# google-research/seed_rl

Hardware: NVIDIA H100
Metric: env-frames/sec (learner, device-timed) on synthetic 84x84x4 T=20 unrolls @1/2/4/8 H100 (higher is better)
Workload: dtype bf16x3 (fp32-faithful tensor-core contraction; activations stored as bf16 hi+lo pairs), f32 elsewhere

## Files before the change

include/seedrl_b200.h:

```cpp
#ifndef SEEDRL_B200_H_
#define SEEDRL_B200_H_

#include <stddef.h>
#include <stdint.h>

#ifdef __cplusplus
extern "C" {
#endif

#define SEEDRL_OK 0
#define SEEDRL_ERR_INVALID_ARGUMENT 3
#define SEEDRL_ERR_OUT_OF_RANGE 11
#define SEEDRL_ERR_INTERNAL 13
#define SEEDRL_ERR_CANCELLED 1
#define SEEDRL_ERR_UNAVAILABLE 14

typedef void* seedrl_stream_t;

const char* seedrl_last_error(void);
int seedrl_abi_version(void);
uint64_t seedrl_kernel_launch_count(void);

int seedrl_vtrace_from_importance_weights(
    int T, int B,
// ... 248 lines not shown
                       const float* B, int ldb, float* C, int ldc, const float* bias,
                       const float* mask, int ldm, int relu, int accumulate, int a_relu,
                       seedrl_stream_t stream);
int seedrl_debug_strided_conv(int op, int mode, int gather, int in_u8, int N, int H, int W, int C, int K,
                              int S, int cout, const void* x, const float* w, const float* bias,
                              const float* dy, const float* mask, float* out, int ldo, float* dbias,
                              float* col, size_t col_bytes, float* ws, size_t ws_bytes, int* error_flag,
                              int* gathered, seedrl_stream_t stream);
size_t seedrl_debug_lstm_workspace_bytes(int mode, int H, int T1, int B);
int seedrl_debug_lstm_forward(int mode, int gemm_mode, int H, int T1, int B, const float* U, const uint8_t* done,
                              float* z, const float* h0, const float* c0, float* hs, float* cs, float* hp,
                              void* ws, size_t ws_bytes, int* error_flag, seedrl_stream_t stream);
int seedrl_debug_lstm_backward(int mode, int gemm_mode, int H, int T1, int B, const float* U, const uint8_t* done,
                               const float* gates, const float* cs, const float* c0, const float* dhs, float* dz,
                               void* ws, size_t ws_bytes, int* error_flag, seedrl_stream_t stream);
int seedrl_debug_r2d2_net_views(const seedrl_r2d2_net* net, int T, int B, int index, size_t* offset, size_t* bytes);
int seedrl_debug_net_views(const seedrl_net* net, int T1, int B, int index, size_t* offset, size_t* bytes,
                           int* format);

size_t seedrl_debug_planes_bytes(int N, int H, int W, int C);
int seedrl_debug_to_planes(int N, int H, int W, int C, int relu, const float* x, void* out,
                           seedrl_stream_t stream);
int seedrl_debug_from_planes(int N, int H, int W, int C, const void* in, float* y,
                             seedrl_stream_t stream);
int seedrl_debug_convp(int cin, int cout, int N, int H, int W, const void* in, const float* w,
                       const float* bias, const void* mask, const void* res, int flip,
                       void* out_raw, void* out_relu, float* out_nhwc, void* wq_scratch,
                       int* error_flag, seedrl_stream_t stream);
int seedrl_debug_wgradp(int cin, int cout, int N, int H, int W, const void* x, const void* dy,
                        float* dw, float* db, float* partial, size_t partial_bytes,
                        int* error_flag, seedrl_stream_t stream);
int seedrl_debug_poolp(int backward, int N, int H, int W, int C, const void* in, void* out_raw,
                       void* out_relu, float* out_nhwc, uint8_t* idx, seedrl_stream_t stream);

#ifdef __cplusplus
}
#endif
#endif
```

seed_rl_b200/_lib.py:

```python
import ctypes
import os

_HERE = os.path.dirname(os.path.abspath(__file__))
LIB_PATH = os.path.join(_HERE, 'libseedrl_b200.so')

c_void_p, c_int, c_float, c_size_t = ctypes.c_void_p, ctypes.c_int, ctypes.c_float, ctypes.c_size_t
c_i64, c_u64 = ctypes.c_int64, ctypes.c_uint64
P = c_void_p


class SeedrlError(RuntimeError):

  def __init__(self, code, msg):
    super().__init__('libseedrl_b200 error %d: %s' % (code, msg))
    self.code = code


class LossConfig(ctypes.Structure):
  _fields_ = [('discounting', c_float), ('lambda_', c_float), ('baseline_cost', c_float),
              ('kl_cost', c_float), ('max_abs_reward', c_float),
              ('clip_rho_threshold', c_float), ('clip_pg_rho_threshold', c_float),
              ('target_entropy', c_float), ('has_target_entropy', ctypes.c_int32),
              ('entropy_cost_adjustment_speed', c_float)]

# ... 95 lines not shown
    'seedrl_r2d2_net_num_params': (c_size_t, [P]),
    'seedrl_r2d2_net_arena_floats': (c_size_t, [P]),
    'seedrl_r2d2_net_set_mode': (c_int, [P, c_int]),
    'seedrl_r2d2_net_set_lstm_mode': (c_int, [P, c_int]),
    'seedrl_r2d2_net_param_info':
        (c_int, [P, c_int, ctypes.c_char_p, c_size_t, ctypes.POINTER(c_i64), ctypes.POINTER(c_int),
                 ctypes.POINTER(c_size_t)]),
    'seedrl_r2d2_net_workspace_bytes': (c_size_t, [P, c_int, c_int]),
    'seedrl_r2d2_net_forward':
        (c_int, [P, P, c_int, c_int, P, P, P, P, P, P, P, P, P, P, P, c_size_t, P]),
    'seedrl_r2d2_net_backward': (c_int, [P, P, c_int, c_int, P, P, P, P, P, c_size_t, P]),
    'seedrl_r2d2_net_check_error': (c_int, [P, c_int, c_int, P, c_size_t, P]),
    'seedrl_r2d2_stack_frames': (c_int, [c_int, c_int, c_int, c_int, P, P, P, P, P, P]),
    'seedrl_r2d2_loss_scratch_bytes': (c_size_t, [c_int, c_int, c_int]),
    'seedrl_r2d2_loss_fwd_bwd': (c_int, [c_int, c_int, c_int, P, P, P, P, P, P, c_float, c_int, c_float, c_float,
                                         P, P, P, P, P]),
    'seedrl_r2d2_retrace_loss_scratch_bytes': (c_size_t, [c_int, c_int]),
    'seedrl_r2d2_retrace_loss_fwd_bwd': (c_int, [c_int, c_int, c_int, P, P, P, P, P, P, c_float, c_float, c_float,
                                                 c_float, P, P, P, P, P]),
    'seedrl_r2d2_epsilon_greedy': (c_int, [c_int, c_int, P, P, c_u64, P, P, P]),
    'seedrl_replay_sample': (c_int, [c_int, P, c_float, c_float, c_int, P, P, P, P, P]),
    'seedrl_clip_scratch_bytes': (c_size_t, []),
    'seedrl_clip_by_global_norm': (c_int, [c_size_t, P, c_float, P, P, P]),
    'seedrl_profile_num_categories': (c_int, []),
    'seedrl_profile_category_name': (ctypes.c_char_p, [c_int]),
    'seedrl_profile_begin': (c_int, [P]),
    'seedrl_profile_end': (c_int, [ctypes.POINTER(ctypes.c_double), ctypes.POINTER(c_u64)]),
    'seedrl_debug_planes_bytes': (c_size_t, [c_int, c_int, c_int, c_int]),
    'seedrl_debug_to_planes': (c_int, [c_int, c_int, c_int, c_int, c_int, P, P, P]),
    'seedrl_debug_from_planes': (c_int, [c_int, c_int, c_int, c_int, P, P, P]),
    'seedrl_debug_convp': (c_int, [c_int, c_int, c_int, c_int, c_int, P, P, P, P, P, c_int, P, P, P, P, P, P]),
    'seedrl_debug_wgradp': (c_int, [c_int, c_int, c_int, c_int, c_int, P, P, P, P, P, c_size_t, P, P]),
    'seedrl_debug_poolp': (c_int, [c_int, c_int, c_int, c_int, c_int, P, P, P, P, P, P]),
    'seedrl_debug_conv3x3': (c_int, [c_int, c_int, c_int, c_int, c_int, c_int, P, P, P, P, P, P, P]),
    'seedrl_debug_conv3x3_flip': (c_int, [c_int, c_int, P, P, P]),
    'seedrl_debug_conv3x3_tc':
        (c_int, [c_int, c_int, c_int, c_int, c_int, c_int, c_int, P, P, P, P, P, P, c_int, c_int, P, P, P]),
    'seedrl_debug_wgrad_partial_bytes': (c_size_t, []),
    'seedrl_debug_conv_pixels': (c_int, [c_int, c_int, c_int, c_int, c_int, c_int, P]),
    'seedrl_debug_set_loss_stream': (c_int, [c_int]),
    'seedrl_debug_set_wgrad_chunk': (c_int, [c_int]),
    'seedrl_debug_set_conv_tile': (c_int, [c_int]),
    'seedrl_debug_set_gemm_bk': (c_int, [c_int]),
    'seedrl_debug_set_first_layer_dense': (c_int, [c_int]),
    'seedrl_debug_conv0pool': (c_int, [c_int, c_int, c_int, P, P, P, P, P, P, P, P]),
    'seedrl_debug_conv0pool_c': (c_int, [c_int, c_int, c_int, c_int, P, P, P, P, P, P, P, P]),
    'seedrl_debug_first_wgrad_pooled_c': (c_int, [c_int, c_int, c_int, c_int, P, P, P, P, P, P, c_size_t, P]),
    'seedrl_debug_conv3x3_wgrad_tc':
        (c_int, [c_int, c_int, c_int, c_int, c_int, c_int, c_int, P, P, P, P, P, c_size_t, P, P]),
    'seedrl_debug_conv3x3_wgrad':
        (c_int, [c_int, c_int, c_int, c_int, c_int, c_int, P, P, P, P, P, c_size_t, P]),
    'seedrl_debug_maxpool': (c_int, [c_int, c_int, c_int, c_int, c_int, P, P, P, P]),
    'seedrl_debug_gemm_tc':
        (c_int, [c_int, c_int, c_int, c_int, c_int, c_int, P, c_int, P, c_int, P, c_int, P, P, c_int, c_int, c_int,
                 c_int, P, c_size_t, P, P]),
    'seedrl_debug_set_gemm_gather': (c_int, [c_int]),
    'seedrl_debug_colsum': (c_int, [c_int, c_int, P, c_int, P, P, c_size_t, P]),
    'seedrl_debug_sgemm':
        (c_int, [c_int, c_int, c_int, c_int, c_int, P, c_int, P, c_int, P, c_int, P, P, c_int,
                 c_int, c_int, c_int, P]),
    'seedrl_debug_strided_conv':
        (c_int, [c_int, c_int, c_int, c_int, c_int, c_int, c_int, c_int, c_int, c_int, c_int, P, P, P, P, P, P,
                 c_int, P, P, c_size_t, P, c_size_t, P, ctypes.POINTER(c_int), P]),
    'seedrl_debug_lstm_workspace_bytes': (c_size_t, [c_int, c_int, c_int, c_int]),
    'seedrl_debug_lstm_forward':
        (c_int, [c_int, c_int, c_int, c_int, c_int, P, P, P, P, P, P, P, P, P, c_size_t, P, P]),
# ... 60 lines not shown
```

seed_rl_b200/csrc/conv_planes.cu:

```cuda
#include <cuda.h>
#include <cuda_bf16.h>

#include <cstdio>
#include <cstdlib>

#include "kernels.h"
#include "tc_common.cuh"

namespace seedrl {

long long planes_positions(int N, int H, int W) {
  const long long Q = (long long)N * (H + 1) * (W + 2);
  return ((Q + 2 * (W + 2) + 2 + 256 + 127) / 128) * 128;
}
size_t planes_bytes(int N, int H, int W, int C) {
  return (size_t)planes_positions(N, H, W) * 16 * 2 * (C / 8);
}

typedef CUresult (*EncodeTiledFn)(CUtensorMap*, CUtensorMapDataType, cuuint32_t, void*, const cuuint64_t*,
                                  const cuuint64_t*, const cuuint32_t*, const cuuint32_t*,
                                  CUtensorMapInterleave, CUtensorMapSwizzle, CUtensorMapL2promotion,
                                  CUtensorMapFloatOOBfill);
static EncodeTiledFn encode_tiled_fn() {
  static EncodeTiledFn fn = nullptr;
// ... 64 lines not shown
  int nch;
  int chunk;
  int ntiles;
  int nb;
  const uint4* wq;
  const float* bias;
  const uint4* mask;
  const uint4* res;
  uint4* out_raw;
  uint4* out_relu;
  float* out_nhwc;
  int* err;
};

constexpr int kCpWarpgroups = 4;
constexpr int kCpThreads = 128 * kCpWarpgroups + 32;
constexpr int kCpM = 128;
constexpr int kCpMaxStages = 4;

__device__ __forceinline__ void quad_transpose(float2 (&t)[4], int q) {
#pragma unroll
  for (int b = 1; b <= 2; b <<= 1) {
    const bool up = (q & b) != 0;
#pragma unroll
    for (int u = 0; u < 4; ++u) {
      if (u & b) continue;
      const float2 send = up ? t[u] : t[u | b];
      const float2 r = make_float2(__shfl_xor_sync(0xffffffffu, send.x, b), __shfl_xor_sync(0xffffffffu, send.y, b));
      if (up) t[u] = r; else t[u | b] = r;
    }
  }
}

template <int CIN, int COUT, int NSUB>
__global__ void __launch_bounds__(kCpThreads, 1)
convp_kernel(const __grid_constant__ CUtensorMap tm_in, const ConvpArgs a) {
  constexpr int G = CIN / 8, GO = COUT / 8, NS = CIN / 16;
  constexpr int MT = NSUB * kCpM;
  constexpr int NBLK = 2 * NSUB;
  extern __shared__ __align__(128) uint8_t smem_raw[];
  const int PW = a.g.PW, nb = a.nb;
  const uint32_t P = (uint32_t)(a.nch * a.chunk) * 16u;
  const uint32_t stage_bytes = 2u * G * P;
  uint8_t* s_stage = smem_raw;
  uint4* s_b = reinterpret_cast<uint4*>(smem_raw + (size_t)nb * stage_bytes);
  float* s_bias = reinterpret_cast<float*>(s_b + 2 * 9 * CIN * COUT / 8);
  uint64_t* s_full = reinterpret_cast<uint64_t*>(s_bias + COUT);
  uint64_t* s_empty = s_full + kCpMaxStages;
  const int tid = threadIdx.x, warp = tid >> 5, lane = tid & 31;

  for (int i = tid; i < 2 * 9 * CIN * COUT / 8; i += kCpThreads) s_b[i] = __ldg(a.wq + i);
  if (tid < COUT) s_bias[tid] = a.bias ? __ldg(a.bias + tid) : 0.f;
  if (tid == 0) {
    for (int i = 0; i < nb; ++i) {
      mbar_init(s_full + i, 1);
      mbar_init(s_empty + i, 4 * kCpWarpgroups);
    }
    asm volatile("fence.mbarrier_init.release.cluster;" ::: "memory");
    asm volatile("prefetch.tensormap [%0];" ::"l"(reinterpret_cast<uint64_t>(&tm_in)) : "memory");
  }
  asm volatile("fence.proxy.async.shared::cta;" ::: "memory");
  __syncthreads();

  const int my_tiles = ((int)blockIdx.x < a.ntiles) ? (a.ntiles - 1 - (int)blockIdx.x) / (int)gridDim.x + 1 : 0;
  bool timed_out = false;

  if (warp == 4 * kCpWarpgroups) {
    if (elect_one()) {
      for (int it = 0; it < my_tiles; ++it) {
        const int s = it % nb;
// ... 1 lines not shown
        const int tile = (int)blockIdx.x + it * (int)gridDim.x;
        mbar_expect_tx(s_full + s, stage_bytes);
        tma_load_3d(s_stage + (size_t)s * stage_bytes, &tm_in, 0, tile * MT / a.chunk, 0, s_full + s);
      }
    }
    __syncwarp();
  } else {
    const int cw = warp >> 2;
    const size_t plane_u = (size_t)a.Lp;
    if (blockIdx.x == 0) {
      const uint4 z = make_uint4(0u, 0u, 0u, 0u);
      for (int i = tid; i < (PW + 1) * 2 * GO; i += 128 * kCpWarpgroups) {
        const int pl = i / (PW + 1), s = i - pl * (PW + 1);
        if (a.out_raw) a.out_raw[(size_t)pl * plane_u + s] = z;
        if (a.out_relu) a.out_relu[(size_t)pl * plane_u + s] = z;
      }
    }
    const int q = lane & 3;
    const int row = 16 * (warp & 3) + (lane >> 2) + 8 * (q & 1);
    const uint32_t b_base = smem_u32(s_b);
    const uint64_t db0 = gmma_desc(b_base, (uint32_t)(2 * GO) * 128u, 128u);
    for (int it = 0; it < my_tiles; ++it) {
      const int s = it % nb;
      const int tile = (int)blockIdx.x + it * (int)gridDim.x;
      if (!mbar_wait_bounded(s_full + s, (uint32_t)((it / nb) & 1))) { timed_out = true; break; }
      const int m0 = (cw - it * NBLK) & (kCpWarpgroups - 1);
      if (m0 >= NBLK && lane == 0) mbar_arrive(s_empty + s);
      const uint32_t a_base = smem_u32(s_stage + (size_t)s * stage_bytes);
      const uint64_t da0 = gmma_desc(a_base, P, 128u);
      const uint64_t lo_off = (uint64_t)((G * P) >> 4), slab_off = (uint64_t)((2 * P) >> 4);
#pragma unroll 1
      for (int m = m0; m < NBLK; m += kCpWarpgroups) {
        float acc[COUT];
#pragma unroll
        for (int i = 0; i < COUT; ++i) acc[i] = 0.f;
        wgmma_fence_acc<COUT>(acc);
        wgmma_fence();
#pragma unroll
        for (int tap = 0; tap < 9; ++tap) {
          const uint64_t off = (uint64_t)(m * 64 + (tap / 3) * PW + (tap % 3));
#pragma unroll
          for (int sl = 0; sl < NS; ++sl) {
            const uint64_t da = da0 + off + (uint64_t)sl * slab_off;
            const uint64_t db = db0 + (uint64_t)((tap * NS + sl) * (COUT * 64 / 16));
            Wgmma<2 * COUT>::template mma<0, 0>(acc, da, db, 1u);
            Wgmma<COUT>::template mma<0, 0>(acc, da + lo_off, db, 1u);
          }
        }
        wgmma_commit();
        const int p = tile * MT + m * 64 + row;
        const int sp = p + PW + 1;
        const int pix = out_pixel(a.g, p);
        uint4 mk[GO / 2], rh[GO / 2], rl[GO / 2];
        if (pix >= 0) {
#pragma unroll
          for (int k = 0; k < GO / 2; ++k) {
            const int go = (q >> 1) + 2 * k;
            if (a.mask) mk[k] = __ldg(a.mask + (size_t)go * plane_u + sp);
            if (a.res) {
              rh[k] = __ldg(a.res + (size_t)go * plane_u + sp);
              rl[k] = __ldg(a.res + (size_t)(GO + go) * plane_u + sp);
            }
          }
        }
        wgmma_wait<0>();
        wgmma_fence_acc<COUT>(acc);
        if (m + kCpWarpgroups >= NBLK && lane == 0) mbar_arrive(s_empty + s);
        const bool in_store = sp < a.Lp;
#pragma unroll
        for (int k = 0; k < GO / 2; ++k) {
          const int go = (q >> 1) + 2 * k;
          float2 t[4];
#pragma unroll
          for (int u = 0; u < 4; ++u) {
            const int j = 2 * k + (u >> 1), h = u & 1;
            t[u] = make_float2(acc[4 * j + 2 * h] + acc[4 * (j + GO) + 2 * h],
                               acc[4 * j + 2 * h + 1] + acc[4 * (j + GO) + 2 * h + 1]);
          }
          quad_transpose(t, q);
          float x[8];
#pragma unroll
          for (int e = 0; e < 4; ++e) {
// ... 320 lines not shown
  if (i >= (long long)Lp * G) return;
  const int s = (int)(i / G), go = (int)(i - (long long)s * G);
  const int pix = in_pixel(g, s);
  if (pix < 0) return;
  const uint4 h = __ldg(in + (size_t)go * Lp + s), l = __ldg(in + (size_t)(G + go) * Lp + s);
  float4* dst = reinterpret_cast<float4*>(y + (size_t)pix * (G * 8) + go * 8);
  dst[0] = make_float4(bf16lo(h.x) + bf16lo(l.x), bf16hi(h.x) + bf16hi(l.x), bf16lo(h.y) + bf16lo(l.y),
                       bf16hi(h.y) + bf16hi(l.y));
  dst[1] = make_float4(bf16lo(h.z) + bf16lo(l.z), bf16hi(h.z) + bf16hi(l.z), bf16lo(h.w) + bf16lo(l.w),
                       bf16hi(h.w) + bf16hi(l.w));
}

int to_planes(int N, int H, int W, int C, int relu, const float* x, void* out, cudaStream_t st) {
  const ConvGeom g = make_geom(N, H, W);
  const long long Lp = planes_positions(N, H, W);
  const long long n = Lp * (C / 8);
  to_planes_kernel<<<(unsigned)((n + 255) / 256), 256, 0, st>>>(g, (int)Lp, C / 8, relu, x,
                                                                reinterpret_cast<uint4*>(out));
  count_launch(PC_MISC, st);
  SEEDRL_CHECK_LAUNCH();
  return SEEDRL_OK;
}
int from_planes(int N, int H, int W, int C, const void* in, float* y, cudaStream_t st) {
  const ConvGeom g = make_geom(N, H, W);
  const long long Lp = planes_positions(N, H, W);
  const long long n = Lp * (C / 8);
  from_planes_kernel<<<(unsigned)((n + 255) / 256), 256, 0, st>>>(g, (int)Lp, C / 8,
                                                                  reinterpret_cast<const uint4*>(in), y);
  count_launch(PC_MISC, st);
  SEEDRL_CHECK_LAUNCH();
  return SEEDRL_OK;
}

__global__ void poolp_fwd_kernel(ConvGeom go_, int Lp, int G, int H, int W, int pt, int pl,
                                 const float* __restrict__ x, uint4* __restrict__ out_raw,
                                 uint4* __restrict__ out_relu, uint8_t* __restrict__ idx) {
  const long long i = (long long)blockIdx.x * blockDim.x + threadIdx.x;
  if (i >= (long long)Lp * G) return;
  const int s = (int)(i / G), gq = (int)(i - (long long)s * G);
  const int pix = in_pixel(go_, s);
  float best[8];
  unsigned char arg[8];
#pragma unroll
  for (int e = 0; e < 8; ++e) { best[e] = 0.f; arg[e] = 0; }
  if (pix >= 0) {
    const int Wo = go_.W, Ho = go_.H, C = G * 8;
    const int n = pix / (Ho * Wo), r = pix - n * (Ho * Wo), ho = r / Wo, wo = r - ho * Wo;
#pragma unroll
    for (int e = 0; e < 8; ++e) best[e] = -INFINITY;
#pragma unroll
    for (int kh = 0; kh < 3; ++kh) {
      const int h = ho * 2 - pt + kh;
      if (h < 0 || h >= H) continue;
#pragma unroll
      for (int kw = 0; kw < 3; ++kw) {
        const int w = wo * 2 - pl + kw;
        if (w < 0 || w >= W) continue;
        const float4* src = reinterpret_cast<const float4*>(x + ((size_t)(n * H + h) * W + w) * C + gq * 8);
        const float4 a = __ldg(src), b = __ldg(src + 1);
        const float v[8] = {a.x, a.y, a.z, a.w, b.x, b.y, b.z, b.w};
        const unsigned char t = (unsigned char)(kh * 3 + kw);
#pragma unroll
        for (int e = 0; e < 8; ++e)
          if (v[e] > best[e]) { best[e] = v[e]; arg[e] = t; }
      }
    }
    uint2 packed;
    packed.x = arg[0] | (arg[1] << 8) | (arg[2] << 16) | ((uint32_t)arg[3] << 24);
    packed.y = arg[4] | (arg[5] << 8) | (arg[6] << 16) | ((uint32_t)arg[7] << 24);
    *reinterpret_cast<uint2*>(idx + (size_t)pix * C + gq * 8) = packed;
  }
  const float4 a = make_float4(best[0], best[1], best[2], best[3]), b = make_float4(best[4], best[5], best[6], best[7]);
  out_raw[(size_t)gq * Lp + s] = pack8_bf16(a, b);
  out_raw[(size_t)(G + gq) * Lp + s] = pack8_bf16(bf16_resid4(a), bf16_resid4(b));
  const float4 ra = make_float4(fmaxf(a.x, 0.f), fmaxf(a.y, 0.f), fmaxf(a.z, 0.f), fmaxf(a.w, 0.f));
  const float4 rb = make_float4(fmaxf(b.x, 0.f), fmaxf(b.y, 0.f), fmaxf(b.z, 0.f), fmaxf(b.w, 0.f));
  out_relu[(size_t)gq * Lp + s] = pack8_bf16(ra, rb);
  out_relu[(size_t)(G + gq) * Lp + s] = pack8_bf16(bf16_resid4(ra), bf16_resid4(rb));
}

template <bool OUT_PLANES>
__global__ void poolp_bwd_kernel(ConvGeom gf, int Lpf, ConvGeom gp, int Lpp, int G, int pt, int pl,
                                 const uint4* __restrict__ dy, const uint8_t* __restrict__ idx,
                                 uint4* __restrict__ dx_planes, float* __restrict__ dx_nhwc) {
  const long long i = (long long)blockIdx.x * blockDim.x + threadIdx.x;
  const int H = gf.H, W = gf.W, Ho = gp.H, Wo = gp.W, C = G * 8;
  int gq, s = 0, pix;
  if (OUT_PLANES) {
    if (i >= (long long)Lpf * G) return;
    s = (int)(i / G); gq = (int)(i - (long long)s * G);
    pix = in_pixel(gf, s);
  } else {
    if (i >= (long long)gf.N * H * W * G) return;
    pix = (int)(i / G); gq = (int)(i - (long long)pix * G);
  }
  float acc[8];
#pragma unroll
  for (int e = 0; e < 8; ++e) acc[e] = 0.f;
  if (pix >= 0) {
    const int n = pix / (H * W), r = pix - n * (H * W), h = r / W, w = r - h * W;
    const int hp = h + pt, wp = w + pl;
#pragma unroll
    for (int dh = 0; dh < 2; ++dh) {
      const int ho = (hp >> 1) - dh;
      const int kh = hp - 2 * ho;
      if (ho < 0 || ho >= Ho || kh > 2) continue;
#pragma unroll
      for (int dw = 0; dw < 2; ++dw) {
        const int wo = (wp >> 1) - dw;
        const int kw = wp - 2 * wo;
        if (wo < 0 || wo >= Wo || kw > 2) continue;
// ... 37 lines not shown
  const ConvGeom g = make_geom(N, Ho, Wo);
  const long long Lp = planes_positions(N, Ho, Wo);
  const long long n = Lp * (C / 8);
  poolp_fwd_kernel<<<(unsigned)((n + 255) / 256), 256, 0, st>>>(g, (int)Lp, C / 8, H, W, pt, pl, x,
                                                                reinterpret_cast<uint4*>(out_raw),
                                                                reinterpret_cast<uint4*>(out_relu), idx);
  count_launch(PC_POOL, st);
  SEEDRL_CHECK_LAUNCH();
  return SEEDRL_OK;
}

int poolp_backward(int N, int H, int W, int C, const void* dy, const uint8_t* idx, void* dx_planes,
                   float* dx_nhwc, cudaStream_t st) {
  int Ho, Wo, pt, pl;
  same_pad3s2(H, &Ho, &pt);
  same_pad3s2(W, &Wo, &pl);
  const ConvGeom gf = make_geom(N, H, W), gp = make_geom(N, Ho, Wo);
  const long long Lpf = planes_positions(N, H, W), Lpp = planes_positions(N, Ho, Wo);
  if (dx_planes) {
    const long long n = Lpf * (C / 8);
    poolp_bwd_kernel<true><<<(unsigned)((n + 255) / 256), 256, 0, st>>>(
        gf, (int)Lpf, gp, (int)Lpp, C / 8, pt, pl, reinterpret_cast<const uint4*>(dy), idx,
        reinterpret_cast<uint4*>(dx_planes), nullptr);
  } else {
    const long long n = (long long)N * H * W * (C / 8);
    poolp_bwd_kernel<false><<<(unsigned)((n + 255) / 256), 256, 0, st>>>(
        gf, (int)Lpf, gp, (int)Lpp, C / 8, pt, pl, reinterpret_cast<const uint4*>(dy), idx, nullptr, dx_nhwc);
  }
  count_launch(PC_POOL, st);
  SEEDRL_CHECK_LAUNCH();
  return SEEDRL_OK;
}

}
```

seed_rl_b200/csrc/kernels.h:

```cpp
#pragma once
#include "common.cuh"

namespace seedrl {

enum { IN_F32 = 0, IN_RELU = 1, IN_U8 = 2 };

struct ConvGeom {
  int N, H, W;
  int PW;
  int RH;
  long long Q;
  unsigned int pw_mul, rh_mul;
  int pw_sh, rh_sh;
};

__host__ __device__ inline void fast_div_setup(unsigned int d, unsigned int* mul, int* sh) {
  int l = 1;
  while ((1u << l) < d) ++l;
  *mul = (unsigned int)(((1ULL << (31 + l)) + d - 1) / d);
  *sh = l - 1;
}
__host__ __device__ __forceinline__ unsigned int fast_div(unsigned int n, unsigned int mul, int sh) {
#ifdef __CUDA_ARCH__
  return __umulhi(n, mul) >> sh;
// ... 45 lines not shown
                     int* err, WgradBatch* batch, cudaStream_t st);
int wgrad_reduce_batch(WgradBatch* b, cudaStream_t st);
int conv3x3_tc_pack_weights_batch(const PackTable& t, int split, cudaStream_t st);
void conv3x3_tc_set_tile(int mt);
int conv3x3_tc_forward(int cin, int cout, int in_mode, int split, int N, int H, int W, const void* in,
                       const void* wq, const float* bias, const float* mask, const float* res,
                       float* out, int variant, int* err, cudaStream_t st);

constexpr int kPlanesTryNext = -12347;
long long planes_positions(int N, int H, int W);
size_t planes_bytes(int N, int H, int W, int C);
struct PlaneConv {
  int N, H, W;
  const void* in;
  const void* wq;
  const float* bias;
  const void* mask;
  const void* res;
  void* out_raw;
  void* out_relu;
  float* out_nhwc;
  int* err;
};
bool convp_supported(int cin, int cout);
int convp_forward(int cin, int cout, const PlaneConv& c, cudaStream_t st);
int wgradp(int cin, int cout, int N, int H, int W, const void* x, const void* dy, float* dw, float* db,
           int* err, WgradBatch* batch, cudaStream_t st);
int to_planes(int N, int H, int W, int C, int relu, const float* x, void* out, cudaStream_t st);
int from_planes(int N, int H, int W, int C, const void* in, float* y, cudaStream_t st);
int poolp_forward(int N, int H, int W, int C, const float* x, void* out_raw, void* out_relu, uint8_t* idx,
                  cudaStream_t st);
int poolp_backward(int N, int H, int W, int C, const void* dy, const uint8_t* idx, void* dx_planes,
                   float* dx_nhwc, cudaStream_t st);

bool first_wgrad_pooled_supported(int cin, int cout, int H, int W);
int first_wgrad_pooled(int N, int H, int W, int C, const uint8_t* frames, const void* g_planes, const uint8_t* idx,
                       float* dw, float* db, WgradBatch* batch, cudaStream_t st);
bool conv0pool_supported(int cin, int cout, int H, int W);
int conv0pool_forward(int N, int H, int W, int C, const uint8_t* frames, const float* w, const float* bias,
                      void* praw, void* prelu, uint8_t* idx, int* err, cudaStream_t st);

int conv3x3_forward(int cin, int cout, int in_mode, int N, int H, int W, const void* in,
                    const float* w, const float* bias, const float* mask, const float* res,
                    float* out, cudaStream_t st);
int conv3x3_u8_forward(int C, int N, int H, int W, const uint8_t* frames, const float* w, const float* bias,
                       float* out, cudaStream_t st);
int conv3x3_u8_wgrad(int C, int N, int H, int W, const uint8_t* frames, const float* dy, float* dw, float* db,
                     float* partial, size_t partial_bytes, cudaStream_t st);
int conv3x3_flip_weights(int cin, int cout, const float* w, float* wt, cudaStream_t st);
size_t conv3x3_wgrad_partial_bytes();
int wgrad_reduce(int nparts, int nw, int nb, const float* partial, float* dw, float* db,
                 cudaStream_t st);
int conv3x3_wgrad(int cin, int cout, int in_mode, int N, int H, int W, const void* x,
                  const float* dy, float* dw, float* db, float* partial, size_t partial_bytes,
                  cudaStream_t st);
int maxpool3s2_forward(int N, int H, int W, int C, const float* x, float* y, uint8_t* idx,
                       cudaStream_t st);
int maxpool3s2_backward(int N, int H, int W, int C, const float* dy, const uint8_t* idx, float* dx,
                        cudaStream_t st);

int convgen_forward(int N, int H, int W, int cin, int cout, int k, int stride, int in_u8,
                    const void* in, const float* w, const float* bias, int relu, float* out,
                    cudaStream_t st);
int convgen_dgrad(int N, int H, int W, int cin, int cout, int k, int stride, const float* dy,
                  const float* w, const float* mask, float* dx, cudaStream_t st);
int convgen_wgrad(int N, int H, int W, int cin, int cout, int k, int stride, int in_u8,
// ... 68 lines not shown
```

seed_rl_b200/csrc/net.cu:

```cuda
#include "schedule.h"

namespace seedrl {

constexpr int kHidden = 256;

struct ConvLayer {
  int cin, cout;
  int w, b;
};
struct Stack {
  int hin, win, cin, c, hout, wout;
  ConvLayer conv, r00, r01, r10, r11;
};

}

struct seedrl_net {
  seedrl_net_config cfg;
  seedrl::ParamTable params;
  size_t logical_params;
  int p_base_w, p_base_b, p_pol_w, p_pol_b;
  seedrl::Core core;
  std::vector<seedrl::Stack> stacks;
  seedrl::StridedConv sh[2];
  int sh_w[2], sh_b[2];
  int conv_mode = 0;
};

namespace seedrl {

static ConvLayer add_conv(seedrl_net* n, const std::string& prefix, int k, int cin, int cout) {
  ConvLayer l;
  l.cin = cin; l.cout = cout;
  l.w = n->params.add(prefix + "/kernel", {k, k, cin, cout});
  l.b = n->params.add(prefix + "/bias", {cout});
  return l;
}

struct StackBufs {
  size_t a0, p, idx, c0, o0, c1, o1;
  size_t praw, prelu, c0r, o0raw, o0relu, c1r, o1p;
};

constexpr size_t kPackSlotBytes = 2 * 9 * 32 * 32 * 2;
constexpr size_t kPartialAllBytes = (size_t)64 << 20;

struct Plan {
  int N;
  std::vector<StackBufs> st;
  size_t sh_a1, sh_a2;
  size_t sh_col0, sh_col1;
  CorePlan core;
  size_t gA, gB, gC, gFull, wt, partial, wq, tcerr, gemm_ws, wq_all, partial_all;
  size_t gP1, gP2, gP3, gFP;
  size_t obs4, w0pad, dw0pad;
  size_t total;
};

static Plan make_plan(const seedrl_net* n, int T1, int B) {
  Plan p;
  Bump b;
  const size_t N = (size_t)T1 * B;
  p.N = (int)N;
  size_t pooled_max = 0, full_max = 0, pooled_planes_max = 0, full_planes_max = 0;
  const bool planes = n->conv_mode == 3 && n->cfg.net == SEEDRL_NET_DEEP;
  if (n->cfg.net == SEEDRL_NET_DEEP) {
    for (size_t si = 0; si < n->stacks.size(); ++si) {
      const Stack& s = n->stacks[si];
      StackBufs sb = StackBufs();
      const size_t full = N * s.hin * s.win * s.c, pooled = N * s.hout * s.wout * s.c;
      sb.a0 = b.take(full * 4);
      sb.idx = b.take(pooled);
      if (!planes) {
        sb.p = b.take(pooled * 4);
        sb.c0 = b.take(pooled * 4);
        sb.o0 = b.take(pooled * 4);
        sb.c1 = b.take(pooled * 4);
        sb.o1 = b.take(pooled * 4);
      } else {
        const size_t pb = planes_bytes((int)N, s.hout, s.wout, s.c);
        sb.praw = b.take(pb); sb.prelu = b.take(pb); sb.c0r = b.take(pb);
        sb.o0raw = b.take(pb); sb.o0relu = b.take(pb); sb.c1r = b.take(pb);
        if (si + 1 < n->stacks.size()) sb.o1p = b.take(pb); else sb.o1 = b.take(pooled * 4);
        if (pb > pooled_planes_max) pooled_planes_max = pb;
        if (si > 0) {
          const size_t fb = planes_bytes((int)N, s.hin, s.win, s.c);
          if (fb > full_planes_max) full_planes_max = fb;
        }
      }
      p.st.push_back(sb);
      if (pooled > pooled_max) pooled_max = pooled;
      if (full > full_max) full_max = full;
    }
    p.sh_a1 = p.sh_a2 = 0;
  } else {
    const StridedConv &l0 = n->sh[0], &l1 = n->sh[1];
    const size_t a1 = N * l0.hout * l0.wout * l0.cout, a2 = N * l1.hout * l1.wout * l1.cout;
    p.sh_a1 = b.take(a1 * 4);
    p.sh_a2 = b.take(a2 * 4);
    p.sh_col0 = p.sh_col1 = 0;
    if (n->conv_mode >= 1) {
      p.sh_col0 = b.take(N * l0.hout * l0.wout * (size_t)(l0.k * l0.k * l0.cin) * 4);
      p.sh_col1 = b.take(N * l1.hout * l1.wout * (size_t)(l1.k * l1.k * l1.cin) * 4);
    }
// ... 285 lines not shown

static int planes_conv(const Call& c, int cin, int cout, int N, int H, int Wd, const void* in, const float* w,
                       int flip, const float* bias, const void* mask, const void* res, void* out_raw, void* out_relu,
                       float* out_nhwc) {
  const void* wq;
  SEEDRL_TRY(packed_weights(c, cin, cout, w, flip, 2, &wq));
  PlaneConv pc;
  pc.N = N; pc.H = H; pc.W = Wd; pc.in = in; pc.wq = wq; pc.bias = bias; pc.mask = mask; pc.res = res;
  pc.out_raw = out_raw; pc.out_relu = out_relu; pc.out_nhwc = out_nhwc; pc.err = c.ex.err;
  return convp_forward(cin, cout, pc, c.ex.st);
}

static int torso_forward_planes(const Call& c, const uint8_t* obs) {
  const seedrl_net* n = c.n; const Plan& pl = c.pl; void* ws = c.ws; cudaStream_t st = c.ex.st;
  const int N = pl.N;
  const void* prev = nullptr;
  const size_t ns = n->stacks.size();
  for (size_t s = 0; s < ns; ++s) {
    const Stack& k = n->stacks[s];
    const StackBufs& b = pl.st[s];
    float* a0 = W<float>(ws, b.a0);
    void* praw = W<void>(ws, b.praw); void* prelu = W<void>(ws, b.prelu);
    void* c0r = W<void>(ws, b.c0r); void* o0raw = W<void>(ws, b.o0raw);
    void* o0relu = W<void>(ws, b.o0relu); void* c1r = W<void>(ws, b.c1r);
    const bool last = s + 1 == ns;
    if (s == 0 && generic_first(n) && g_first_dense)
      return set_error(SEEDRL_ERR_INVALID_ARGUMENT,
                       "the dense first-layer path takes 3- or 4-channel frames; switch it off for these frames");
    if (s == 0 && conv0pool_supported(first_c(n), k.c, k.hin, k.win) && !g_first_dense) {
      SEEDRL_TRY(conv0pool_forward(N, k.hin, k.win, first_c(n), obs, c.P(k.conv.w), c.P(k.conv.b), praw,
                                   prelu, W<uint8_t>(ws, b.idx), W<int>(ws, pl.tcerr), st));
    } else if (s == 0 && generic_first(n)) {
      return set_error(SEEDRL_ERR_INVALID_ARGUMENT, "conv mode 3: the fused first layer takes frames up to 107 pixels wide");
    } else {
      if (s == 0)
        SEEDRL_TRY(run_conv(c, k.cin, k.c, IN_U8, N, k.hin, k.win, obs, c.P(k.conv.w),
                            c.P(k.conv.b), nullptr, nullptr, a0, 0));
      else
        SEEDRL_TRY(planes_conv(c, k.cin, k.c, N, k.hin, k.win, prev, c.P(k.conv.w), 0,
                               c.P(k.conv.b), nullptr, nullptr, nullptr, nullptr, a0));
      SEEDRL_TRY(poolp_forward(N, k.hin, k.win, k.c, a0, praw, prelu, W<uint8_t>(ws, b.idx), st));
    }
    const int H = k.hout, Wd = k.wout, C = k.c;
    SEEDRL_TRY(planes_conv(c, C, C, N, H, Wd, prelu, c.P(k.r00.w), 0, c.P(k.r00.b), nullptr,
                           nullptr, nullptr, c0r, nullptr));
    SEEDRL_TRY(planes_conv(c, C, C, N, H, Wd, c0r, c.P(k.r01.w), 0, c.P(k.r01.b), nullptr,
                           praw, o0raw, o0relu, nullptr));
    SEEDRL_TRY(planes_conv(c, C, C, N, H, Wd, o0relu, c.P(k.r10.w), 0, c.P(k.r10.b), nullptr,
                           nullptr, nullptr, c1r, nullptr));
    SEEDRL_TRY(planes_conv(c, C, C, N, H, Wd, c1r, c.P(k.r11.w), 0, c.P(k.r11.b), nullptr,
                           o0raw, last ? nullptr : W<void>(ws, b.o1p), nullptr,
                           last ? W<float>(ws, b.o1) : nullptr));
    prev = W<void>(ws, b.o1p);
  }
  return SEEDRL_OK;
}

static int torso_forward_shallow(const Call& c, const uint8_t* obs) {
  const seedrl_net* n = c.n; const Plan& pl = c.pl; void* ws = c.ws; cudaStream_t st = c.ex.st;
  const int N = pl.N;
  float* a1 = W<float>(ws, pl.sh_a1);
  float* a2 = W<float>(ws, pl.sh_a2);
  if (n->conv_mode >= 1 && n->cfg.obs_c % 4 == 0) {
    SEEDRL_TRY(n->sh[0].forward(c.ex, N, true, obs, c.P(n->sh_w[0]), c.P(n->sh_b[0]), W<float>(ws, pl.sh_col0), a1,
                                16));
    return n->sh[1].forward(c.ex, N, false, a1, c.P(n->sh_w[1]), c.P(n->sh_b[1]), W<float>(ws, pl.sh_col1), a2, 32);
// ... 400 lines not shown
}
extern "C" int seedrl_debug_from_planes(int N, int H, int W, int C, const void* in, float* y,
                                        seedrl_stream_t stream) {
  SEEDRL_CHECK_ARG(N >= 1 && H >= 1 && W >= 1 && C >= 8 && C % 8 == 0 && in && y, "bad arguments");
  return from_planes(N, H, W, C, in, y, (cudaStream_t)stream);
}
extern "C" int seedrl_debug_convp(int cin, int cout, int N, int H, int W, const void* in, const float* w,
                                  const float* bias, const void* mask, const void* res, int flip,
                                  void* out_raw, void* out_relu, float* out_nhwc, void* wq_scratch,
                                  int* error_flag, seedrl_stream_t stream) {
  SEEDRL_CHECK_ARG(convp_supported(cin, cout) && in && w && wq_scratch, "unsupported (cin,cout) or null pointer");
  SEEDRL_TRY(conv3x3_tc_pack_weights(cin, cout, flip, 2, w, wq_scratch, (cudaStream_t)stream));
  PlaneConv c;
  c.N = N; c.H = H; c.W = W; c.in = in; c.wq = wq_scratch; c.bias = bias; c.mask = mask; c.res = res;
  c.out_raw = out_raw; c.out_relu = out_relu; c.out_nhwc = out_nhwc; c.err = error_flag;
  return convp_forward(cin, cout, c, (cudaStream_t)stream);
}
extern "C" int seedrl_debug_wgradp(int cin, int cout, int N, int H, int W, const void* x, const void* dy,
                                   float* dw, float* db, float* partial, size_t partial_bytes,
                                   int* error_flag, seedrl_stream_t stream) {
  SEEDRL_CHECK_ARG(x && dy && dw && db && partial, "null pointer");
  WgradBatch wb{partial, partial_bytes / sizeof(float), 0, 0, {}};
  SEEDRL_TRY(wgradp(cin, cout, N, H, W, x, dy, dw, db, error_flag, &wb, (cudaStream_t)stream));
  return wgrad_reduce_batch(&wb, (cudaStream_t)stream);
}
extern "C" int seedrl_debug_poolp(int backward, int N, int H, int W, int C, const void* in, void* out_raw,
                                  void* out_relu, float* out_nhwc, uint8_t* idx, seedrl_stream_t stream) {
  SEEDRL_CHECK_ARG(N >= 1 && H >= 1 && W >= 1 && C >= 8 && C % 8 == 0 && in && idx, "bad arguments");
  if (backward) return poolp_backward(N, H, W, C, in, idx, out_raw, out_nhwc, (cudaStream_t)stream);
  SEEDRL_CHECK_ARG(out_raw && out_relu, "null pointer");
  return poolp_forward(N, H, W, C, reinterpret_cast<const float*>(in), out_raw, out_relu, idx,
                       (cudaStream_t)stream);
}
```

Measured before the change: 198,600.

## Fuse stack conv with 3x3 stride-2 max-pool in a banded TMA/wgmma kernel

```diff
diff --git a/include/seedrl_b200.h b/include/seedrl_b200.h
--- a/include/seedrl_b200.h
+++ b/include/seedrl_b200.h
@@ -304,6 +304,9 @@
                         int* error_flag, seedrl_stream_t stream);
 int seedrl_debug_poolp(int backward, int N, int H, int W, int C, const void* in, void* out_raw,
                        void* out_relu, float* out_nhwc, uint8_t* idx, seedrl_stream_t stream);
+int seedrl_debug_convp_pool(int cin, int cout, int N, int H, int W, const void* in, const float* w,
+                            const float* bias, void* out_raw, void* out_relu, uint8_t* idx, void* wq_scratch,
+                            int* error_flag, seedrl_stream_t stream);
 
 #ifdef __cplusplus
 }
diff --git a/seed_rl_b200/_lib.py b/seed_rl_b200/_lib.py
--- a/seed_rl_b200/_lib.py
+++ b/seed_rl_b200/_lib.py
@@ -151,6 +151,7 @@
     'seedrl_debug_convp': (c_int, [c_int, c_int, c_int, c_int, c_int, P, P, P, P, P, c_int, P, P, P, P, P, P]),
     'seedrl_debug_wgradp': (c_int, [c_int, c_int, c_int, c_int, c_int, P, P, P, P, P, c_size_t, P, P]),
     'seedrl_debug_poolp': (c_int, [c_int, c_int, c_int, c_int, c_int, P, P, P, P, P, P]),
+    'seedrl_debug_convp_pool': (c_int, [c_int, c_int, c_int, c_int, c_int, P, P, P, P, P, P, P, P, P]),
     'seedrl_debug_conv3x3': (c_int, [c_int, c_int, c_int, c_int, c_int, c_int, P, P, P, P, P, P, P]),
     'seedrl_debug_conv3x3_flip': (c_int, [c_int, c_int, P, P, P]),
     'seedrl_debug_conv3x3_tc':
diff --git a/seed_rl_b200/csrc/conv_planes.cu b/seed_rl_b200/csrc/conv_planes.cu
--- a/seed_rl_b200/csrc/conv_planes.cu
+++ b/seed_rl_b200/csrc/conv_planes.cu
@@ -120,10 +120,32 @@
   }
 }
 
+template <int CIN, int COUT>
+__device__ __forceinline__ void convp_block_mma(float (&acc)[COUT], uint64_t da0, uint64_t db0, int base, int PW,
+                                                uint64_t lo_off, uint64_t slab_off) {
+  constexpr int NS = CIN / 16;
+#pragma unroll
+  for (int i = 0; i < COUT; ++i) acc[i] = 0.f;
+  wgmma_fence_acc<COUT>(acc);
+  wgmma_fence();
+#pragma unroll
+  for (int tap = 0; tap < 9; ++tap) {
+    const uint64_t off = (uint64_t)(base + (tap / 3) * PW + (tap % 3));
+#pragma unroll
+    for (int sl = 0; sl < NS; ++sl) {
+      const uint64_t da = da0 + off + (uint64_t)sl * slab_off;
+      const uint64_t db = db0 + (uint64_t)((tap * NS + sl) * (COUT * 64 / 16));
+      Wgmma<2 * COUT>::template mma<0, 0>(acc, da, db, 1u);
+      Wgmma<COUT>::template mma<0, 0>(acc, da + lo_off, db, 1u);
+    }
+  }
+  wgmma_commit();
+}
+
 template <int CIN, int COUT, int NSUB>
 __global__ void __launch_bounds__(kCpThreads, 1)
 convp_kernel(const __grid_constant__ CUtensorMap tm_in, const ConvpArgs a) {
-  constexpr int G = CIN / 8, GO = COUT / 8, NS = CIN / 16;
+  constexpr int G = CIN / 8, GO = COUT / 8;
   constexpr int MT = NSUB * kCpM;
   constexpr int NBLK = 2 * NSUB;
   extern __shared__ __align__(128) uint8_t smem_raw[];
@@ -191,22 +213,7 @@
 #pragma unroll 1
       for (int m = m0; m < NBLK; m += kCpWarpgroups) {
         float acc[COUT];
-#pragma unroll
-        for (int i = 0; i < COUT; ++i) acc[i] = 0.f;
-        wgmma_fence_acc<COUT>(acc);
-        wgmma_fence();
-#pragma unroll
-        for (int tap = 0; tap < 9; ++tap) {
-          const uint64_t off = (uint64_t)(m * 64 + (tap / 3) * PW + (tap % 3));
-#pragma unroll
-          for (int sl = 0; sl < NS; ++sl) {
-            const uint64_t da = da0 + off + (uint64_t)sl * slab_off;
-            const uint64_t db = db0 + (uint64_t)((tap * NS + sl) * (COUT * 64 / 16));
-            Wgmma<2 * COUT>::template mma<0, 0>(acc, da, db, 1u);
-            Wgmma<COUT>::template mma<0, 0>(acc, da + lo_off, db, 1u);
-          }
-        }
-        wgmma_commit();
+        convp_block_mma<CIN, COUT>(acc, da0, db0, m * 64, PW, lo_off, slab_off);
         const int p = tile * MT + m * 64 + row;
         const int sp = p + PW + 1;
         const int pix = out_pixel(a.g, p);
@@ -593,6 +600,45 @@
   return SEEDRL_OK;
 }
 
+template <typename Load>
+__device__ __forceinline__ uint2 pool3s2_window8(int h0, int w0, int H, int W, Load ld, float (&best)[8]) {
+  unsigned char arg[8];
+#pragma unroll
+  for (int e = 0; e < 8; ++e) { best[e] = -INFINITY; arg[e] = 0; }
+#pragma unroll
+  for (int kh = 0; kh < 3; ++kh) {
+    const int h = h0 + kh;
+    if (h < 0 || h >= H) continue;
+#pragma unroll
+    for (int kw = 0; kw < 3; ++kw) {
+      const int w = w0 + kw;
+      if (w < 0 || w >= W) continue;
+      float4 a, b;
+      ld(h, w, a, b);
+      const float v[8] = {a.x, a.y, a.z, a.w, b.x, b.y, b.z, b.w};
+      const unsigned char t = (unsigned char)(kh * 3 + kw);
+#pragma unroll
+      for (int e = 0; e < 8; ++e)
+        if (v[e] > best[e]) { best[e] = v[e]; arg[e] = t; }
+    }
+  }
+  uint2 packed;
+  packed.x = arg[0] | (arg[1] << 8) | (arg[2] << 16) | ((uint32_t)arg[3] << 24);
+  packed.y = arg[4] | (arg[5] << 8) | (arg[6] << 16) | ((uint32_t)arg[7] << 24);
+  return packed;
+}
+
+__device__ __forceinline__ void store_pooled8(const float (&v)[8], uint4* out_raw, uint4* out_relu, size_t Lp, int G,
+                                              int gq, int s) {
+  const float4 a = make_float4(v[0], v[1], v[2], v[3]), b = make_float4(v[4], v[5], v[6], v[7]);
+  out_raw[(size_t)gq * Lp + s] = pack8_bf16(a, b);
+  out_raw[(size_t)(G + gq) * Lp + s] = pack8_bf16(bf16_resid4(a), bf16_resid4(b));
+  const float4 ra = make_float4(fmaxf(a.x, 0.f), fmaxf(a.y, 0.f), fmaxf(a.z, 0.f), fmaxf(a.w, 0.f));
+  const float4 rb = make_float4(fmaxf(b.x, 0.f), fmaxf(b.y, 0.f), fmaxf(b.z, 0.f), fmaxf(b.w, 0.f));
+  out_relu[(size_t)gq * Lp + s] = pack8_bf16(ra, rb);
+  out_relu[(size_t)(G + gq) * Lp + s] = pack8_bf16(bf16_resid4(ra), bf16_resid4(rb));
+}
+
 __global__ void poolp_fwd_kernel(ConvGeom go_, int Lp, int G, int H, int W, int pt, int pl,
                                  const float* __restrict__ x, uint4* __restrict__ out_raw,
                                  uint4* __restrict__ out_relu, uint8_t* __restrict__ idx) {
@@ -601,43 +647,18 @@
   const int s = (int)(i / G), gq = (int)(i - (long long)s * G);
   const int pix = in_pixel(go_, s);
   float best[8];
-  unsigned char arg[8];
-#pragma unroll
-  for (int e = 0; e < 8; ++e) { best[e] = 0.f; arg[e] = 0; }
+#pragma unroll
+  for (int e = 0; e < 8; ++e) best[e] = 0.f;
   if (pix >= 0) {
     const int Wo = go_.W, Ho = go_.H, C = G * 8;
     const int n = pix / (Ho * Wo), r = pix - n * (Ho * Wo), ho = r / Wo, wo = r - ho * Wo;
-#pragma unroll
-    for (int e = 0; e < 8; ++e) best[e] = -INFINITY;
-#pragma unroll
-    for (int kh = 0; kh < 3; ++kh) {
-      const int h = ho * 2 - pt + kh;
-      if (h < 0 || h >= H) continue;
-#pragma unroll
-      for (int kw = 0; kw < 3; ++kw) {
-        const int w = wo * 2 - pl + kw;
-        if (w < 0 || w >= W) continue;
-        const float4* src = reinterpret_cast<const float4*>(x + ((size_t)(n * H + h) * W + w) * C + gq * 8);
-        const float4 a = __ldg(src), b = __ldg(src + 1);
-        const float v[8] = {a.x, a.y, a.z, a.w, b.x, b.y, b.z, b.w};
-        const unsigned char t = (unsigned char)(kh * 3 + kw);
-#pragma unroll
-        for (int e = 0; e < 8; ++e)
-          if (v[e] > best[e]) { best[e] = v[e]; arg[e] = t; }
-      }
-    }
-    uint2 packed;
-    packed.x = arg[0] | (arg[1] << 8) | (arg[2] << 16) | ((uint32_t)arg[3] << 24);
-    packed.y = arg[4] | (arg[5] << 8) | (arg[6] << 16) | ((uint32_t)arg[7] << 24);
-    *reinterpret_cast<uint2*>(idx + (size_t)pix * C + gq * 8) = packed;
-  }
-  const float4 a = make_float4(best[0], best[1], best[2], best[3]), b = make_float4(best[4], best[5], best[6], best[7]);
-  out_raw[(size_t)gq * Lp + s] = pack8_bf16(a, b);
-  out_raw[(size_t)(G + gq) * Lp + s] = pack8_bf16(bf16_resid4(a), bf16_resid4(b));
-  const float4 ra = make_float4(fmaxf(a.x, 0.f), fmaxf(a.y, 0.f), fmaxf(a.z, 0.f), fmaxf(a.w, 0.f));
-  const float4 rb = make_float4(fmaxf(b.x, 0.f), fmaxf(b.y, 0.f), fmaxf(b.z, 0.f), fmaxf(b.w, 0.f));
-  out_relu[(size_t)gq * Lp + s] = pack8_bf16(ra, rb);
-  out_relu[(size_t)(G + gq) * Lp + s] = pack8_bf16(bf16_resid4(ra), bf16_resid4(rb));
+    auto ld = [&](int h, int w, float4& a, float4& b) {
+      const float4* src = reinterpret_cast<const float4*>(x + ((size_t)(n * H + h) * W + w) * C + gq * 8);
+      a = __ldg(src); b = __ldg(src + 1);
+    };
+    *reinterpret_cast<uint2*>(idx + (size_t)pix * C + gq * 8) = pool3s2_window8(ho * 2 - pt, wo * 2 - pl, H, W, ld, best);
+  }
+  store_pooled8(best, out_raw, out_relu, Lp, G, gq, s);
 }
 
 template <bool OUT_PLANES>
@@ -741,4 +762,229 @@
   return SEEDRL_OK;
 }
 
-}
+struct ConvpPoolArgs {
+  ConvGeom g;
+  int Ho, Wo, pt, pl;
+  int Lpp, PWp, RHp;
+  int k, bands;
+  int srows;
+  const uint4* wq;
+  const float* bias;
+  uint4* out_raw; uint4* out_relu;
+  uint8_t* idx;
+  int* err;
+};
+
+constexpr size_t kCppHeader = 256;
+constexpr int kCppStages = 3;
+__host__ __device__ constexpr int convp_pool_band_stride(int cout) { return cout + 4; }
+
+__device__ __forceinline__ void mma_threads_sync() {
+  asm volatile("bar.sync 1, %0;" ::"n"(128 * kCpWarpgroups) : "memory");
+}
+
+template <int CIN, int COUT>
+__global__ void __launch_bounds__(kCpThreads, 1)
+convp_pool_kernel(const __grid_constant__ CUtensorMap tm_in, const ConvpPoolArgs a) {
+  constexpr int G = CIN / 8, GO = COUT / 8, SB = convp_pool_band_stride(COUT);
+  constexpr int WB = 2 * 9 * CIN * COUT * 2;
+  extern __shared__ __align__(128) uint8_t smem_raw[];
+  const int PW = a.g.PW, H = a.g.H, W = a.g.W;
+  const uint32_t P = (uint32_t)(a.srows * PW) * 16u;
+  const uint32_t stage_bytes = 2u * G * P, stage_pitch = (stage_bytes + 127u) & ~127u;
+  uint4* s_b = reinterpret_cast<uint4*>(smem_raw);
+  float* s_bias = reinterpret_cast<float*>(smem_raw + WB);
+  uint64_t* s_full = reinterpret_cast<uint64_t*>(smem_raw + WB + 128);
+  uint64_t* s_empty = s_full + kCppStages;
+  uint8_t* s_stage = smem_raw + WB + kCppHeader;
+  float* s_band = reinterpret_cast<float*>(s_stage + (size_t)kCppStages * stage_pitch);
+  const int tid = threadIdx.x, warp = tid >> 5, lane = tid & 31;
+
+  for (int i = tid; i < WB / 16; i += kCpThreads) s_b[i] = __ldg(a.wq + i);
+  if (tid < COUT) s_bias[tid] = __ldg(a.bias + tid);
+  if (tid == 0) {
+    for (int i = 0; i < kCppStages; ++i) {
+      mbar_init(s_full + i, 1);
+      mbar_init(s_empty + i, 4 * kCpWarpgroups);
+    }
+    asm volatile("fence.mbarrier_init.release.cluster;" ::: "memory");
+    asm volatile("prefetch.tensormap [%0];" ::"l"(reinterpret_cast<uint64_t>(&tm_in)) : "memory");
+  }
+  asm volatile("fence.proxy.async.shared::cta;" ::: "memory");
+  __syncthreads();
+
+  const int units = a.g.N * a.bands;
+  const int my_units = ((int)blockIdx.x < units) ? (units - 1 - (int)blockIdx.x) / (int)gridDim.x + 1 : 0;
+  auto band_of = [&](int u, int& n, int& r0, int& r1, int& cr0, int& cr1) {
+    n = u / a.bands;
+    r0 = (u - n * a.bands) * a.k;
+    r1 = min(a.Ho, r0 + a.k);
+    cr0 = max(0, 2 * r0 - a.pt);
+    cr1 = min(H - 1, 2 * (r1 - 1) - a.pt + 2);
+  };
+  bool timed_out = false;
+
+  if (warp == 4 * kCpWarpgroups) {
+    if (elect_one()) {
+      for (int it = 0; it < my_units; ++it) {
+        const int s = it % kCppStages;
+        if (it >= kCppStages && !mbar_wait_bounded(s_empty + s, (uint32_t)(((it / kCppStages) - 1) & 1))) { timed_out = true; break; }
+        int n, r0, r1, cr0, cr1;
+        band_of((int)blockIdx.x + it * (int)gridDim.x, n, r0, r1, cr0, cr1);
+        mbar_expect_tx(s_full + s, stage_bytes);
+        tma_load_3d(s_stage + (size_t)s * stage_pitch, &tm_in, 0, n * a.g.RH + cr0, 0, s_full + s);
+      }
+    }
+    __syncwarp();
+  } else {
+    const int cw = warp >> 2;
+    const size_t plane_p = (size_t)a.Lpp;
+    const uint4 z = make_uint4(0u, 0u, 0u, 0u);
+    auto zero_padding = [&](int u) {
+      int n, r0, r1, cr0, cr1;
+      band_of(u, n, r0, r1, cr0, cr1);
+      const int n_side = 2 * (r1 - r0), n_top = r0 == 0 ? a.PWp : 0;
+      const int t0 = a.g.N * a.RHp * a.PWp, n_tail = u == units - 1 ? a.Lpp - t0 : 0;
+      for (int i = tid; i < (n_side + n_top + n_tail) * 2 * GO; i += 128 * kCpWarpgroups) {
+        const int pl_ = i % (2 * GO), j = i / (2 * GO);
+        const int sp = j < n_side ? (n * a.RHp + r0 + (j >> 1) + 1) * a.PWp + ((j & 1) ? a.Wo + 1 : 0)
+                     : j < n_side + n_top ? n * a.RHp * a.PWp + (j - n_side)
+                     : t0 + (j - n_side - n_top);
+        a.out_raw[pl_ * plane_p + sp] = z;
+        a.out_relu[pl_ * plane_p + sp] = z;
+      }
+    };
+    auto pool_band = [&](int u) {
+      mma_threads_sync();
+      int n, r0, r1, cr0, cr1;
+      band_of(u, n, r0, r1, cr0, cr1);
+      const int nq = (r1 - r0) * a.Wo;
+      for (int i = tid; i < nq * GO; i += 128 * kCpWarpgroups) {
+        const int gq = i % GO, qq = i / GO;
+        const int qr = qq / a.Wo, qw = qq - qr * a.Wo, qh = r0 + qr;
+        auto ld = [&](int h, int w, float4& x0, float4& x1) {
+          const float4* p = reinterpret_cast<const float4*>(s_band + ((h - cr0) * PW + w) * SB + gq * 8);
+          x0 = p[0]; x1 = p[1];
+        };
+        float best[8];
+        const uint2 taps = pool3s2_window8(qh * 2 - a.pt, qw * 2 - a.pl, H, W, ld, best);
+        *reinterpret_cast<uint2*>(a.idx + ((size_t)(n * a.Ho + qh) * a.Wo + qw) * COUT + gq * 8) = taps;
+        store_pooled8(best, a.out_raw, a.out_relu, plane_p, GO, gq, (n * a.RHp + qh + 1) * a.PWp + qw + 1);
+      }
+      mma_threads_sync();
+    };
+
+    const int q = lane & 3;
+    const int row = 16 * (warp & 3) + (lane >> 2);
+    const uint64_t db0 = gmma_desc(smem_u32(s_b), (uint32_t)(2 * GO) * 128u, 128u);
+    const uint64_t lo_off = (uint64_t)((G * P) >> 4), slab_off = (uint64_t)((2 * P) >> 4);
+    for (int it = 0; it < my_units; ++it) {
+      const int s = it % kCppStages;
+      const int u = (int)blockIdx.x + it * (int)gridDim.x;
+      int n, r0, r1, cr0, cr1;
+      band_of(u, n, r0, r1, cr0, cr1);
+      const int npos = (cr1 - cr0 + 1) * PW, nblk = (npos + 63) >> 6;
+      zero_padding(u);
+      if (!timed_out && !mbar_wait_bounded(s_full + s, (uint32_t)((it / kCppStages) & 1))) timed_out = true;
+      if (cw >= nblk && lane == 0) mbar_arrive(s_empty + s);
+      const uint64_t da0 = gmma_desc(smem_u32(s_stage + (size_t)s * stage_pitch), P, 128u);
+      bool pooled = it == 0;
+#pragma unroll 1
+      for (int m = cw; m < nblk; m += kCpWarpgroups) {
+        float acc[COUT];
+        convp_block_mma<CIN, COUT>(acc, da0, db0, m * 64, PW, lo_off, slab_off);
+        if (!pooled) { pool_band(u - (int)gridDim.x); pooled = true; }
+        wgmma_wait<0>();
+        wgmma_fence_acc<COUT>(acc);
+        if (m + kCpWarpgroups >= nblk && lane == 0) mbar_arrive(s_empty + s);
+#pragma unroll
+        for (int h = 0; h < 2; ++h) {
+          const int o = m * 64 + row + 8 * h;
+          if (o < npos) {
+#pragma unroll
+            for (int j = 0; j < GO; ++j) {
+              const int c = 8 * j + 2 * q;
+              *reinterpret_cast<float2*>(s_band + o * SB + c) =
+                  make_float2(acc[4 * j + 2 * h] + acc[4 * (j + GO) + 2 * h] + s_bias[c],
+                              acc[4 * j + 2 * h + 1] + acc[4 * (j + GO) + 2 * h + 1] + s_bias[c + 1]);
+            }
+          }
+        }
+      }
+      if (!pooled) pool_band(u - (int)gridDim.x);
+    }
+    if (my_units > 0) pool_band((int)blockIdx.x + (my_units - 1) * (int)gridDim.x);
+  }
+  if (timed_out && a.err) atomicExch(a.err, 1);
+}
+
+static size_t convp_pool_smem(int cin, int cout, int H, int W, int k, int* srows) {
+  const int PW = W + 2;
+  const int cr = 2 * k + 1 < H ? 2 * k + 1 : H;
+  const int nblk = (cr * PW + 63) / 64;
+  *srows = (nblk * 64 + 2 * PW + 2 + PW - 1) / PW;
+  const size_t stage = ((size_t)2 * (cin / 8) * *srows * PW * 16 + 127) / 128 * 128;
+  return (size_t)2 * 9 * cin * cout * 2 + kCppHeader + kCppStages * stage + (size_t)cr * PW * convp_pool_band_stride(cout) * 4;
+}
+
+static int convp_pool_rows(int cin, int cout, int H, int W, int* srows) {
+  int Ho, pt;
+  same_pad3s2(H, &Ho, &pt);
+  if (W + 2 > 128) return 0;
+  for (int k = Ho; k >= 1; --k)
+    if (convp_pool_smem(cin, cout, H, W, k, srows) <= 227 * 1024 && *srows <= 256) return k;
+  return 0;
+}
+
+bool convp_pool_supported(int cin, int cout, int H, int W) {
+  int srows;
+  return ((cin == 16 && cout == 32) || (cin == 32 && cout == 32)) && H >= 1 && W >= 1 &&
+         convp_pool_rows(cin, cout, H, W, &srows) > 0;
+}
+
+template <int CIN, int COUT>
+static int launch_convp_pool(ConvpPoolArgs a, const void* in, cudaStream_t st) {
+  const ConvGeom& g = a.g;
+  const long long Lp = planes_positions(g.N, g.H, g.W);
+  int dummy;
+  const size_t smem = convp_pool_smem(CIN, COUT, g.H, g.W, a.k, &dummy);
+  CUtensorMap tm;
+  SEEDRL_TRY(make_plane_map(&tm, in, Lp, 2 * (CIN / 8), 0, g.PW, a.srows, 2 * (CIN / 8)));
+  static bool attr = false;
+  if (!attr) {
+    SEEDRL_CUDA(cudaFuncSetAttribute(convp_pool_kernel<CIN, COUT>, cudaFuncAttributeMaxDynamicSharedMemorySize,
+                                     227 * 1024));
+    attr = true;
+  }
+  static const bool dbg = getenv("SEEDRL_DEBUG_LAUNCH") != nullptr;
+  if (dbg) fprintf(stderr, "convp_pool<%d,%d> H=%d W=%d k=%d srows=%d smem=%zu\n", CIN, COUT, g.H, g.W, a.k, a.srows,
+                   smem);
+  const int units = g.N * a.bands;
+  const int grid = units < kNumSMs ? units : kNumSMs;
+  convp_pool_kernel<CIN, COUT><<<grid, kCpThreads, smem, st>>>(tm, a);
+  count_launch(PC_CONV_FWD, st);
+  SEEDRL_CHECK_LAUNCH();
+  return SEEDRL_OK;
+}
+
+int convp_pool_forward(int cin, int cout, int N, int H, int W, const void* in, const void* wq, const float* bias,
+                       void* out_raw, void* out_relu, uint8_t* idx, int* err, cudaStream_t st) {
+  if (!convp_pool_supported(cin, cout, H, W) || N < 1)
+    return set_error(SEEDRL_ERR_INVALID_ARGUMENT, "convp_pool: unsupported (cin, cout) or image too wide");
+  if (planes_positions(N, H, W) >= (1LL << 31))
+    return set_error(SEEDRL_ERR_INVALID_ARGUMENT, "convp_pool: batch too large for 32-bit positions");
+  ConvpPoolArgs a;
+  a.k = convp_pool_rows(cin, cout, H, W, &a.srows);
+  a.g = make_geom(N, H, W);
+  same_pad3s2(H, &a.Ho, &a.pt);
+  same_pad3s2(W, &a.Wo, &a.pl);
+  a.Lpp = (int)planes_positions(N, a.Ho, a.Wo); a.PWp = a.Wo + 2; a.RHp = a.Ho + 1;
+  a.bands = (a.Ho + a.k - 1) / a.k;
+  a.wq = reinterpret_cast<const uint4*>(wq); a.bias = bias;
+  a.out_raw = reinterpret_cast<uint4*>(out_raw); a.out_relu = reinterpret_cast<uint4*>(out_relu);
+  a.idx = idx; a.err = err;
+  if (cin == 16) return launch_convp_pool<16, 32>(a, in, st);
+  return launch_convp_pool<32, 32>(a, in, st);
+}
+
+}
diff --git a/seed_rl_b200/csrc/kernels.h b/seed_rl_b200/csrc/kernels.h
--- a/seed_rl_b200/csrc/kernels.h
+++ b/seed_rl_b200/csrc/kernels.h
@@ -101,6 +101,9 @@
                   cudaStream_t st);
 int poolp_backward(int N, int H, int W, int C, const void* dy, const uint8_t* idx, void* dx_planes,
                    float* dx_nhwc, cudaStream_t st);
+bool convp_pool_supported(int cin, int cout, int H, int W);
+int convp_pool_forward(int cin, int cout, int N, int H, int W, const void* in, const void* wq, const float* bias,
+                       void* out_raw, void* out_relu, uint8_t* idx, int* err, cudaStream_t st);
 
 bool first_wgrad_pooled_supported(int cin, int cout, int H, int W);
 int first_wgrad_pooled(int N, int H, int W, int C, const uint8_t* frames, const void* g_planes, const uint8_t* idx,
diff --git a/seed_rl_b200/csrc/net.cu b/seed_rl_b200/csrc/net.cu
--- a/seed_rl_b200/csrc/net.cu
+++ b/seed_rl_b200/csrc/net.cu
@@ -56,6 +56,10 @@
   size_t obs4, w0pad, dw0pad;
   size_t total;
 };
+
+static bool stack_conv_pooled(const Stack& s, size_t si) {
+  return si > 0 && convp_pool_supported(s.cin, s.c, s.hin, s.win);
+}
 
 static Plan make_plan(const seedrl_net* n, int T1, int B) {
   Plan p;
@@ -69,7 +73,7 @@
       const Stack& s = n->stacks[si];
       StackBufs sb = StackBufs();
       const size_t full = N * s.hin * s.win * s.c, pooled = N * s.hout * s.wout * s.c;
-      sb.a0 = b.take(full * 4);
+      sb.a0 = planes && stack_conv_pooled(s, si) ? 0 : b.take(full * 4);
       sb.idx = b.take(pooled);
       if (!planes) {
         sb.p = b.take(pooled * 4);
@@ -421,6 +425,11 @@
                                    prelu, W<uint8_t>(ws, b.idx), W<int>(ws, pl.tcerr), st));
     } else if (s == 0 && generic_first(n)) {
       return set_error(SEEDRL_ERR_INVALID_ARGUMENT, "conv mode 3: the fused first layer takes frames up to 107 pixels wide");
+    } else if (stack_conv_pooled(k, s)) {
+      const void* wq;
+      SEEDRL_TRY(packed_weights(c, k.cin, k.c, c.P(k.conv.w), 0, 2, &wq));
+      SEEDRL_TRY(convp_pool_forward(k.cin, k.c, N, k.hin, k.win, prev, wq, c.P(k.conv.b), praw, prelu,
+                                    W<uint8_t>(ws, b.idx), c.ex.err, st));
     } else {
       if (s == 0)
         SEEDRL_TRY(run_conv(c, k.cin, k.c, IN_U8, N, k.hin, k.win, obs, c.P(k.conv.w),
@@ -887,3 +896,12 @@
   return poolp_forward(N, H, W, C, reinterpret_cast<const float*>(in), out_raw, out_relu, idx,
                        (cudaStream_t)stream);
 }
+extern "C" int seedrl_debug_convp_pool(int cin, int cout, int N, int H, int W, const void* in, const float* w,
+                                       const float* bias, void* out_raw, void* out_relu, uint8_t* idx,
+                                       void* wq_scratch, int* error_flag, seedrl_stream_t stream) {
+  SEEDRL_CHECK_ARG(N >= 1 && in && w && bias && out_raw && out_relu && idx && wq_scratch, "bad arguments");
+  SEEDRL_CHECK_ARG(convp_pool_supported(cin, cout, H, W), "unsupported (cin, cout) or image too wide");
+  SEEDRL_TRY(conv3x3_tc_pack_weights(cin, cout, 0, 2, w, wq_scratch, (cudaStream_t)stream));
+  return convp_pool_forward(cin, cout, N, H, W, in, wq_scratch, bias, out_raw, out_relu, idx, error_flag,
+                            (cudaStream_t)stream);
+}
```

Result: faster. 203,100, median of 6 (+2.3%).
